# terasum/mythril

Measured on AMD Instinct MI355X. Metric: constraint-evals/sec, higher is better.
Workload: dtype u32; 1 GPU; synthetic config 5: 10000 random 256-bit constraint tapes x 67108864 assignments per GPU, throughput mode; variant=plain, tapes=10000, rows_per_gpu=67108864, rows_total=67108864, vars=4, mode=count_all, engine=jit, short_circuit=True, parallelism=dp1 (row shards, all-reduce of per-tape results)

## Files before the change

### mythril_amd/csrc/jit.cpp

```cpp
#include "jit.h"

#include <math.h>
#include <stdarg.h>
#include <stdio.h>
#include <string.h>

#include <algorithm>
#include <atomic>
#include <climits>
#include <cstdlib>
#include <functional>
#include <stdexcept>
#include <string>
#include <thread>
#include <unordered_map>
#include <vector>

namespace mh {
namespace jit {

namespace {

struct Fail {
    std::string why;
// ... 64 lines not shown
uint32_t prefix_mask(uint32_t m) { int t = top_bit(m); return t < 0 ? 0u : ((2u << t) - 1u); }

class Emitter {
public:
    Emitter(const SsaTape& st, const std::vector<uint32_t>& pool, uint32_t n_vars,
            const Options& opt, const std::vector<uint8_t>* check = nullptr,
            std::vector<double>* insn_cost = nullptr)
        : st_(st), pool_(pool), n_vars_(n_vars), opt_(opt), check_(check),
          insn_cost_(insn_cost) {}

    TapeCode run();

private:
    SsaTape st_;
    const std::vector<uint32_t>& pool_;
    uint32_t n_vars_;
    Options opt_;
    const std::vector<uint8_t>* check_;
    std::vector<double>* insn_cost_;
    bool sc_used_ = false;
    std::vector<MI> code_;
    std::vector<Val> vals_;
    std::vector<int> last_;
    std::vector<uint8_t> dem_;
    int vref_[512] = {};
    uint32_t vbase_ = 0, vmax_ = 0, vhigh_ = 0;
    int pref_[N_BOOL_PAIRS] = {};
    uint32_t kstage_ = 0;
    uint32_t n_valu_ = 0, n_wide_ = 0, n_salu_ = 0;
    uint32_t n_valu_cold_ = 0;
    int cold_ = 0;
    bool calls_div_ = false;
    bool calls_divw_ = false;
    bool uses_lds_ = false;
    bool calls_kec_ = false;
    int cur_op_ = -1;
    int live_vreg_ = -1;
public:
    static uint64_t op_valu[256], op_wide[256], op_count[256];
    int div_ = 0;
    bool divw_ = false;
private:

    void emit(uint16_t op, std::initializer_list<Opnd> ops, bool e64 = false) {
        MI m;
        m.op = op;
        m.e64 = e64 ? 1 : 0;
        m.tag = cur_op_ >= 0 ? (uint8_t)cur_op_ : 0xFF;
        int i = 0;
        for (const Opnd& o : ops) m.o[i++] = o;
        code_.push_back(m);
        if (op <= M_V_CMP_LE_F64) {
            ++n_valu_;
            if (cold_ > 0) ++n_valu_cold_;
            const bool wide = e64 || op == M_V_ADD_CO || op == M_V_ADDC_CO || op == M_V_SUB_CO ||
                              op == M_V_SUBB_CO || op == M_V_SUBREV_CO || op == M_V_SUBBREV_CO ||
                              op == M_V_OR3 || op == M_V_ALIGNBIT || op == M_V_MAD_U64_U32 ||
                              op == M_V_LSHL_ADD || op == M_V_PERM || op == M_V_BFI ||
                              op == M_V_LSHLREV || op == M_V_LSHRREV || op == M_V_ASHRREV ||
                              (op >= M_V_CMP_EQ && op <= M_V_CMP_GT_I32) || op >= M_V_CVT_F64_U32 ||
                              op == M_V_RCP_F32 || op == M_V_CMP_GT_F32 || op == M_V_CMP_LE_F32;
            if (wide) ++n_wide_;
            if (cur_op_ >= 0) { ++op_valu[cur_op_]; op_wide[cur_op_] += wide; }
        } else if (op <= M_S_CMP_LT_U32) {
            ++n_salu_;
        }
    }

    uint32_t next_lbl_ = 0x1000;

    uint32_t valloc() {
        for (uint32_t r = vbase_; r < vmax_; ++r)
            if (vref_[r] == 0) {
                vref_[r] = 1;
// ... 1186 lines not shown
    const uint32_t rbase = kind == 1 ? R_DR : R_DQ;
    int path = 0;
    if (div_ >= 1 && ny >= 1 && nx < ny && kind < 4) {
        if (kind < 2 && B.l[ny - 1].is_c()) {
            Val R;
            R.defined = true;
            for (int k = 0; k < 8; ++k) {
                if (!((dm >> k) & 1)) continue;
                R.l[k] = kind == 1 && k < nx ? A.l[k] : Limb::C(0);
                if (R.l[k].is_r()) vretain(R.l[k].v);
            }
            vals_[d] = R;
            return;
        }
        path = B.l[ny - 1].is_r() ? 1 : 0;
        if (kind & 1)
            for (int k = 0; k < nx; ++k)
                if (A.l[k].is_r() && A.l[k].v >= rbase && A.l[k].v < rbase + 8 &&
                    A.l[k].v != rbase + (uint32_t)k)
                    path = 0;
    } else if (div_ >= 3 && nx == 8 && ny == 8 && (kind == 0 || kind == 2)) {
        path = 3;
    }
    uint32_t l_join = 0;
    if (path) {
        const uint32_t l_cold = next_lbl_++;
        l_join = next_lbl_++;
        if (path == 1) div_short_dividend(A, B, kind, nx, dm, cur, l_cold);
        else div_small_quotient(A, B, kind, dm, cur, l_cold);
        emit(M_S_BRANCH, {LBL(l_join)});
        emit(M_LABEL, {LBL(l_cold)});
        ++cold_;
    }
    if (kind < 2) {
        for (int k = 0; k < 8; ++k) emit(M_V_MOV, {V(R_DY + k), src(B.l[k])});
        for (int k = 0; k < 8; ++k) emit(M_V_MOV, {V(R_DR + k), src(A.l[k])});
    } else {
        auto sign_of = [&](const Val& X, uint32_t sreg) {
            if (X.l[7].is_c()) emit(M_V_MOV, {V(sreg), IMM((X.l[7].v >> 31) ? ~0u : 0u)});
            else emit(M_V_ASHRREV, {V(sreg), IMM(31), V(X.l[7].v)});
        };
        auto load_abs = [&](uint32_t base, uint32_t sreg, const Val& X) {
            bool allc = true;
            for (int k = 0; k < 8; ++k) allc = allc && X.l[k].is_c();
            const bool known = X.l[7].is_c(), neg = known && (X.l[7].v >> 31);
            if (allc) {
                uint32_t c[8];
                uint64_t borrow = neg ? 1 : 0;
                for (int k = 0; k < 8; ++k) {
                    const uint64_t t = (uint64_t)(neg ? ~X.l[k].v : X.l[k].v) + borrow;
                    c[k] = (uint32_t)t;
                    borrow = t >> 32;
                }
                for (int k = 0; k < 8; ++k) emit(M_V_MOV, {V(base + k), IMM(c[k])});
                return;
            }
            if (known && !neg) {
                for (int k = 0; k < 8; ++k) emit(M_V_MOV, {V(base + k), src(X.l[k])});
                return;
            }
            for (int k = 0; k < 8; ++k) {
                if (X.l[k].is_c(0)) emit(M_V_MOV, {V(base + k), V(sreg)});
                else emit(M_V_XOR, {V(base + k), src(X.l[k]), V(sreg)});
            }
            emit(M_V_SUB_CO, {V(base), VCC(), V(base), V(sreg)});
            for (int k = 1; k < 8; ++k)
                emit(M_V_SUBB_CO, {V(base + k), VCC(), V(base + k), V(sreg), VCC()});
// ... 4 lines not shown
        load_abs(R_DR, R_SX, A);
    }
    int wny = 0;
    bool wconst = false;
    uint32_t yc[8] = {0};
    if (divw_ && path == 0) {
        wconst = true;
        for (int k = 0; k < 8; ++k) wconst = wconst && B.l[k].is_c();
        if (wconst) {
            const bool neg = kind >= 2 && (B.l[7].v >> 31);
            uint64_t carry = neg ? 1 : 0;
            for (int k = 0; k < 8; ++k) {
                const uint64_t t = (uint64_t)(neg ? ~B.l[k].v : B.l[k].v) + carry;
                yc[k] = (uint32_t)t;
                carry = t >> 32;
            }
            wny = 8;
            while (wny > 0 && !yc[wny - 1]) --wny;
        } else {
            wny = ny;
        }
        if (wny < 1 || wny > 7 || nx < wny) wny = 0;
    }
    if (wny) {
        const int j0 = nx - wny;
        calls_divw_ = true;
        emit(M_S_MOV_B32, {S(S_DIV_KIND), IMM(kind | (uint32_t)((wconst ? 64 : 0) + 8 * wny + j0) << 3)});
        emit(M_S_MOV_B32, {S(S_DIV_DUMMY), IMM(kind)});
        if (wconst) {
            const uint64_t rb = div_recip_bits(yc, wny);
            emit(M_S_MOV_B32, {S(S_DIV_F64K), IMM((uint32_t)rb)});
            emit(M_S_MOV_B32, {S(S_DIV_F64K + 1), IMM((uint32_t)(rb >> 32))});
        }
    } else {
        emit(M_S_MOV_B32, {S(S_DIV_KIND), IMM(kind)});
    }
    emit(M_CALL_DIV, {IMM((uint32_t)code_.size())});
    if (path) {
        --cold_;
        emit(M_LABEL, {LBL(l_join)});
    }
    int nr = path == 1 && (kind & 1) ? nx : 8;
    if (wny && wconst && kind < 2) nr = kind == 1 ? wny : nx - wny + 1;
    Val& R = out(d);
    for (int k = 0; k < 8; ++k)
        if ((dm >> k) & 1) R.l[k] = k < nr ? Limb::R(rbase + k) : Limb::C(0);
}

void Emitter::div_undecided(Opnd decided, int cur) {
    const Opnd t = S(S_DIV_TM, 2);
    emit(M_S_ANDN2_B64, {t, S(S_VALID, 2), decided});
    const int lv = live_vreg_;
    if (check_ && lv >= 0 && vals_[lv].defined && vals_[lv].is_bool && vals_[lv].bconst < 0 &&
        last_[lv] > cur)
        emit(M_S_AND_B64, {t, t, P(vals_[lv].pair)});
}

void Emitter::div_short_dividend(const Val& A, const Val& B, uint32_t kind, int nx, uint32_t dm,
                                 int cur, uint32_t l_cold) {
    int ny = 8;
    while (!B.l[ny - 1].is_r()) --ny;
    const uint32_t top = B.l[ny - 1].v;
    if (kind < 2) {
        emit(M_V_CMP_NE, {VCC(), IMM(0), V(top)});
    } else {
        emit(M_V_ASHRREV, {V(R_T1), IMM(31), V(top)});
        emit(M_V_XOR, {V(R_T1), V(top), V(R_T1)});
        emit(M_V_CMP_NE, {VCC(), IMM(0), V(R_T1)});
    }
// ... 881 lines not shown
                emit(M_S_BRANCH, {LBL(LBL_SC_END)});
                emit(M_LABEL, {LBL(LBL_SC_SKIP)});
                emit(M_S_MOV_B64, {S(S_RES, 2), IMM(0)});
                emit(M_LABEL, {LBL(LBL_SC_END)});
            }
            for (int k = 0; k < 8; ++k) { tc.root_limbs[k] = ~0u; tc.root_const[k] = 0; }
        } else {
            uint32_t acc = ~0u, cacc = 0;
            for (int k = 0; k < 8; ++k) {
                const Limb l = root.l[k];
                if (l.is_c()) { cacc |= l.v; tc.root_limbs[k] = ~0u; tc.root_const[k] = l.v; continue; }
                tc.root_limbs[k] = l.v;
                tc.root_const[k] = 0;
                if (acc == ~0u) { acc = valloc(); emit(M_V_MOV, {V(acc), V(l.v)}); }
                else emit(M_V_OR, {V(acc), V(l.v), V(acc)});
            }
            if (cacc) emit(M_S_MOV_B64, {S(S_RES, 2), IMM(~0u)});
            else if (acc == ~0u) emit(M_S_MOV_B64, {S(S_RES, 2), IMM(0)});
            else {
                emit(M_V_CMP_NE, {VCC(), IMM(0), V(acc)});
                emit(M_S_MOV_B64, {S(S_RES, 2), VCC()});
            }
        }
        tc.ok = true;
    } catch (const Fail& f) {
        tc.ok = false;
        tc.why = f.why;
        code_.clear();
    }
    tc.code.swap(code_);
    tc.max_vgpr = vhigh_;
    tc.calls_div = calls_div_;
    tc.calls_divw = calls_divw_;
    tc.uses_lds = uses_lds_;
    tc.calls_kec = calls_kec_;
    tc.n_valu = n_valu_;
    tc.n_valu_wide = n_wide_;
    tc.n_salu = n_salu_;
    return tc;
}

struct OpInfo {
    const char* name;
};
const char* op_name(uint16_t op) {
    switch (op) {
        case M_V_MOV: return "v_mov_b32";
        case M_V_ADD_U32: return "v_add_u32";
        case M_V_SUB_U32: return "v_sub_u32";
        case M_V_SUBREV_U32: return "v_subrev_u32";
        case M_V_ADD_CO: return "v_add_co_u32";
        case M_V_ADDC_CO: return "v_addc_co_u32";
        case M_V_SUB_CO: return "v_sub_co_u32";
        case M_V_SUBB_CO: return "v_subb_co_u32";
        case M_V_SUBREV_CO: return "v_subrev_co_u32";
        case M_V_SUBBREV_CO: return "v_subbrev_co_u32";
        case M_V_AND: return "v_and_b32";
        case M_V_OR: return "v_or_b32";
        case M_V_XOR: return "v_xor_b32";
        case M_V_NOT: return "v_not_b32";
        case M_V_XNOR: return "v_xnor_b32";
        case M_V_OR3: return "v_or3_b32";
        case M_V_ALIGNBIT: return "v_alignbit_b32";
        case M_V_LSHLREV: return "v_lshlrev_b32";
        case M_V_LSHRREV: return "v_lshrrev_b32";
        case M_V_ASHRREV: return "v_ashrrev_i32";
// ... 90 lines not shown
        for (const Opnd& x : ops) m.o[i++] = x;
        o.push_back(m);
    };
    auto L = [&](uint32_t id) { E(M_LABEL, {LBL(id)}); };
    auto Yr = [](int k) { return V(R_DY + k); };
    auto Rr = [](int k) { return V(R_DR + k); };
    auto Xr = [](int k) { return V(R_DQ + k); };
    const Opnd FY = V(R_FY, 2), FR = V(R_FR, 2), FC = V(R_FC, 2), FT = V(R_FT, 2);
    const Opnd CARRY = V(R_CARRY, 2), MAD = V(R_MAD, 2);
    const Opnd C = V(R_C), T1 = V(R_T1), SX = V(R_SX), SY = V(R_SY);
    const Opnd YNZ = S(S_DIV_YNZ, 2), DUMMY = S(S_DIV_DUMMY, 2), MSK = S(S_DIV_MSK, 2),
               TM = S(S_DIV_TM, 2), K64 = S(S_DIV_F64K, 2), KIND = S(S_DIV_KIND);
    const Opnd K64LO = S(S_DIV_F64K), K64HI = S(S_DIV_F64K + 1);
    enum : uint32_t { L_UNS = 1, L_DONE, L_TOP3, L_CONV, L_ZQ, L_NOZQ, L_STEP0 = 10, L_NONEG0 = 20, L_NOGE0 = 30, L_WB = 40,
                      L_SDIV, L_SREM, L_SMOD, L_NARROW = 50, L_NNEG0 = 60, L_NGE0 = 70,
                      L_NOYZ = 80, L_CZ0 = 90, L_RLT = 100, L_RLTD, L_YSLOW, L_YDONE, L_TOPALL,
                      L_F32 = 110, L_F32OK, L_STEP0_BODY };
    auto to_f64 = [&](Opnd dst, Opnd (*limb)(int)) {
        E(M_S_MOV_B32, {K64LO, IMM(0)});
        E(M_S_MOV_B32, {K64HI, IMM(0x41f00000u)});
        E(M_V_CVT_F64_U32, {dst, limb(7)});
        for (int k = 6; k >= 0; --k) {
            E(M_V_CVT_F64_U32, {FT, limb(k)});
            E(M_V_FMA_F64, {dst, dst, K64, FT});
        }
    };
    auto Rl = [](int k) { return V(R_DR + k); };
    auto Yl = [](int k) { return V(R_DY + k); };
    const Opnd KEEP = S(S_DIV_DUMMY);
    enum : uint32_t { L_WHEAD = 128, L_WSEC, L_WCONST, L_WVAR = 136 , L_WCON = 144 ,
                      L_WOK = 152 , L_WZQ = 160 ,
                      L_WSTEP = 256 , L_WNONEG = 384, L_WNOGE = 512,
                      L_WTREE = 640 };
    L(L_WHEAD);
    E(M_S_CMP_LT_U32, {KIND, IMM(64)});
    E(M_S_CBRANCH_SCC1, {LBL(L_UNS)});
    {
        uint32_t tree = L_WTREE;
        std::function<void(int, int, uint32_t, uint32_t)> pick = [&](int lo, int hi, uint32_t c,
                                                                      uint32_t base) {
            if (lo == hi) {
                E(M_S_BRANCH, {LBL(base + (uint32_t)lo)});
                return;
            }
            const int mid = (lo + hi + 1) / 2;
            const uint32_t l = tree++;
            E(M_S_CMP_LT_U32, {KIND, IMM((64 * c + 8 * (uint32_t)mid) << 3)});
            E(M_S_CBRANCH_SCC0, {LBL(l)});
            pick(lo, mid - 1, c, base);
            L(l);
            pick(mid, hi, c, base);
        };
        E(M_S_CMP_LT_U32, {KIND, IMM(64u << 3)});
        E(M_S_CBRANCH_SCC0, {LBL(L_WCONST)});
        pick(1, 7, 0, L_WVAR);
        L(L_WCONST);
        pick(1, 7, 1, L_WCON);
    }
    L(L_UNS);
    E(M_S_CMP_EQ_U32, {KIND, IMM(0)});
    E(M_S_CBRANCH_SCC1, {LBL(L_ZQ)});
    E(M_S_CMP_EQ_U32, {KIND, IMM(2)});
    E(M_S_CBRANCH_SCC0, {LBL(L_NOZQ)});
    L(L_ZQ);
    for (int k = 0; k < 8; ++k) E(M_V_MOV, {Xr(k), IMM(0)});
    L(L_NOZQ);
// ... 17 lines not shown
    E(M_V_CMP_LT, {VCC(), Rr(7), Yr(7)});
    E(M_S_BRANCH, {LBL(L_RLTD)});
    L(L_RLT);
    E(M_V_SUB_CO, {T1, VCC(), Rr(0), Yr(0)});
    for (int k = 1; k < 8; ++k) E(M_V_SUBB_CO, {T1, VCC(), Rr(k), Yr(k), VCC()});
    L(L_RLTD);
    E(M_S_ANDN2_B64, {MSK, YNZ, VCC()});
    E(M_S_CMP_EQ_U64, {MSK, IMM(0)});
    E(M_S_CBRANCH_SCC1, {LBL(L_DONE)});
    E(M_S_CMP_EQ_U64, {TM, IMM(0)});
    E(M_S_CBRANCH_SCC1, {LBL(L_NARROW)});
    auto recip = [&]() {
        E(M_V_RCP_F64, {FC, FY});
        E(M_S_NOP, {IMM(1)});
        E(M_V_FMA_F64, {FT, NEG(FY), FC, FONE()});
        E(M_V_FMA_F64, {FC, FC, FT, FC});
        E(M_V_FMA_F64, {FT, NEG(FY), FC, FONE()});
        E(M_V_FMA_F64, {FY, FC, FT, FC});
    };
    auto top3_f64 = [&](Opnd dst, Opnd (*limb)(int)) {
        E(M_S_MOV_B32, {K64LO, IMM(0)});
        E(M_S_MOV_B32, {K64HI, IMM(0x41f00000u)});
        E(M_V_CVT_F64_U32, {dst, limb(7)});
        for (int k = 6; k >= 5; --k) {
            E(M_V_CVT_F64_U32, {FT, limb(k)});
            E(M_V_FMA_F64, {dst, dst, K64, FT});
        }
        E(M_S_MOV_B32, {K64HI, IMM((uint32_t)(1023 + 160) << 20)});
        E(M_V_MUL_F64, {dst, dst, K64});
    };
    E(M_V_CMP_NE, {VCC(), IMM(0), Yr(7)});
    E(M_S_ANDN2_B64, {TM, MSK, VCC()});
    E(M_S_CBRANCH_SCC0, {LBL(L_F32)});
    to_f64(FY, Yl);
    recip();
    to_f64(FR, Rl);
    E(M_S_BRANCH, {LBL(L_CONV)});
    L(L_F32);
    E(M_S_MOV_B32, {K64LO, IMM(0x4f800000u)});
    E(M_V_CVT_F32_U32, {V(R_FT), Rr(7)});
    E(M_V_CVT_F32_U32, {V(R_FT + 1), Rr(6)});
    E(M_V_FMA_F32, {V(R_FR), V(R_FT), K64LO, V(R_FT + 1)});
    E(M_V_CVT_F32_U32, {V(R_FT), Yr(7)});
    E(M_V_CVT_F32_U32, {V(R_FT + 1), Yr(6)});
    E(M_V_FMA_F32, {V(R_FY), V(R_FT), K64LO, V(R_FT + 1)});
    E(M_V_RCP_F32, {V(R_FY), V(R_FY)});
    E(M_S_NOP, {IMM(1)});
    E(M_V_MUL_F32, {V(R_FC), V(R_FR), V(R_FY)});
    E(M_V_CMP_GT_F32, {VCC(), IMM(0x44800000u), V(R_FC)});
    E(M_S_ANDN2_B64, {TM, MSK, VCC()});
    E(M_S_CBRANCH_SCC0, {LBL(L_F32OK)});
    E(M_V_CMP_NE, {VCC(), IMM(0), Yr(7)});
    E(M_S_BRANCH, {LBL(L_TOP3)});
    L(L_F32OK);
    E(M_V_CVT_U32_F32, {C, V(R_FC)});
    E(M_V_CNDMASK, {C, IMM(0), C, MSK}, true);
    E(M_V_FRACT_F32, {V(R_FT), V(R_FC)});
    E(M_V_CMP_LE_F32, {VCC(), IMM(0x3f7f8000u), V(R_FT)});
    E(M_S_AND_B64, {TM, VCC(), MSK});
    E(M_S_BRANCH, {LBL(L_STEP0_BODY)});
    L(L_TOP3);
    top3_f64(FY, Yl);
    recip();
    E(M_S_CMP_EQ_U64, {VCC(), IMM(0xFFFFFFFFu)});
    E(M_S_CBRANCH_SCC1, {LBL(L_TOPALL)});
    E(M_V_CNDMASK, {V(R_FY), IMM(0), V(R_FY), MSK}, true);
// ... 321 lines not shown
            E(M_S_MOV_B64, {MSK, VCC()});
            E(M_S_CMP_EQ_U64, {MSK, IMM(0)});
            E(M_S_CBRANCH_SCC1, {LBL(L_WNONEG + id)});
            for (int k = 0; k < ny; ++k) {
                E(M_V_CNDMASK, {T1, IMM(0), Yr(k), MSK}, true);
                if (k == 0) E(M_V_ADD_CO, {Rr(j), VCC(), Rr(j), T1});
                else E(M_V_ADDC_CO, {Rr(j + k), VCC(), Rr(j + k), T1, VCC()});
            }
            if (top <= 7) E(M_V_ADDC_CO, {Rr(top), VCC(), IMM(0), Rr(top), VCC()});
            E(M_V_CNDMASK, {T1, IMM(0), IMM(1), MSK}, true);
            E(M_V_SUB_U32, {C, C, T1});
            L(L_WNONEG + id);
            E(M_S_CMP_EQ_U64, {TM, IMM(0)});
            E(M_S_CBRANCH_SCC1, {LBL(L_WNOGE + id)});
            E(M_V_SUB_CO, {T1, VCC(), Rr(j), Yr(0)});
            for (int k = 1; k < ny; ++k) E(M_V_SUBB_CO, {T1, VCC(), Rr(j + k), Yr(k), VCC()});
            if (top <= 7) E(M_V_SUBBREV_CO, {T1, VCC(), IMM(0), Rr(top), VCC()});
            E(M_S_ANDN2_B64, {MSK, YNZ, VCC()});
            E(M_S_CMP_EQ_U64, {MSK, IMM(0)});
            E(M_S_CBRANCH_SCC1, {LBL(L_WNOGE + id)});
            for (int k = 0; k < ny; ++k) {
                E(M_V_CNDMASK, {T1, IMM(0), Yr(k), MSK}, true);
                if (k == 0) E(M_V_SUB_CO, {Rr(j), VCC(), Rr(j), T1});
                else E(M_V_SUBB_CO, {Rr(j + k), VCC(), Rr(j + k), T1, VCC()});
            }
            if (top <= 7) E(M_V_SUBBREV_CO, {Rr(top), VCC(), IMM(0), Rr(top), VCC()});
            E(M_V_CNDMASK, {T1, IMM(0), IMM(1), MSK}, true);
            E(M_V_ADD_U32, {C, C, T1});
            L(L_WNOGE + id);
            E(M_V_MOV, {Xr(j), C});
        }
        leave(L_DONE);
    }
    return o;
}

namespace {
const uint64_t kKeccakRC[24] = {
    0x0000000000000001ull, 0x0000000000008082ull, 0x800000000000808Aull, 0x8000000080008000ull,
    0x000000000000808Bull, 0x0000000080000001ull, 0x8000000080008081ull, 0x8000000000008009ull,
    0x000000000000008Aull, 0x0000000000000088ull, 0x0000000080008009ull, 0x000000008000000Aull,
    0x000000008000808Bull, 0x800000000000008Bull, 0x8000000000008089ull, 0x8000000000008003ull,
    0x8000000000008002ull, 0x8000000000000080ull, 0x000000000000800Aull, 0x800000008000000Aull,
    0x8000000080008081ull, 0x8000000000008080ull, 0x0000000080000001ull, 0x8000000080008008ull};
const int kRhoPi[24][2] = {{10, 1}, {7, 3},   {11, 6},  {17, 10}, {18, 15}, {3, 21},
                           {5, 28}, {16, 36}, {8, 45},  {21, 55}, {24, 2},  {4, 14},
                           {15, 27}, {23, 41}, {19, 56}, {13, 8},  {12, 25}, {2, 43},
                           {20, 62}, {14, 18}, {22, 39}, {9, 61},  {6, 20},  {1, 44}};
}

namespace {

void kec_theta_states(uint8_t* comp) {
    uint8_t c[5] = {0}, d[5];
    for (int i = 0; i < 25; ++i) c[i % 5] ^= comp[i];
    for (int x = 0; x < 5; ++x) d[x] = c[(x + 4) % 5] ^ c[(x + 1) % 5];
    for (int i = 0; i < 25; ++i) comp[i] ^= d[i % 5];
}

void kec_rhopi_states(uint8_t* comp) {
    uint8_t cur = comp[1];
    for (int step = 0; step < 24; ++step) {
        const int dst = kRhoPi[step][0];
        const uint8_t t = comp[dst];
        comp[dst] = cur;
        cur = t;
// ... 324 lines not shown
    char b[512];
    va_list ap;
    va_start(ap, fmt);
    vsnprintf(b, sizeof b, fmt, ap);
    va_end(ap);
    out += b;
    out += '\n';
}

}

Module build_module(const std::vector<const TapeCode*>& codes,
                    const std::vector<uint32_t>& tape_ids, uint32_t n_vars, bool values,
                    uint32_t group_bytes) {
    Module m;
    std::string& o = m.text;
    uint32_t cur = 0, first = 0;
    for (uint32_t i = 0; i < codes.size(); ++i) {
        const uint32_t b = code_bytes(*codes[i]) + 96;
        if (i > first && (cur + b > group_bytes || i - first >= 64)) {
            m.group_first.push_back(first);
            m.group_count.push_back(i - first);
            first = i;
            cur = 0;
        }
        cur += b;
    }
    if (first < codes.size()) {
        m.group_first.push_back(first);
        m.group_count.push_back((uint32_t)codes.size() - first);
    }
    const uint32_t n_pin = pinned_cols(n_vars);
    uint32_t maxv = R_COL0 + 8 * n_pin;
    bool any_div = false, any_divw = false, any_lds = false, any_kec = false;
    for (const TapeCode* tc : codes) {
        maxv = std::max(maxv, tc->max_vgpr);
        any_div |= tc->calls_div;
        any_divw |= tc->calls_divw;
        any_lds |= tc->uses_lds;
        any_kec |= tc->calls_kec;
    }
    if (any_kec) maxv = std::max<uint32_t>(maxv, R_TEMP_KEC);
    if (any_div) maxv = std::max<uint32_t>(maxv, R_TEMP0);
    maxv = std::max<uint32_t>(maxv, 8);
    static const uint32_t pad = [] {
        const char* e = std::getenv("MH_JIT_PAD_VGPR");
        const uint32_t v = e ? (uint32_t)atoi(e) : 0u;
        return v <= 512 ? v : 0u;
    }();
    maxv = std::max(maxv, pad);
    maxv = (maxv + 7) & ~7u;
    m.max_vgpr = maxv;
    m.n_sgpr = S_NEXT_FREE;

    line(o, ".amdgcn_target \"amdgcn-amd-amdhsa--gfx950\"");
    line(o, ".amdhsa_code_object_version 5");
    line(o, ".text");
    line(o, ".globl mh_jit");
    line(o, ".p2align 8");
    line(o, ".type mh_jit,@function");
    line(o, "mh_jit:");
    line(o, "s_load_dwordx16 s[4:19], s[0:1], 0x0");
    line(o, "s_load_dwordx4 s[20:23], s[0:1], 0x40");
    line(o, "v_and_b32 v1, 63, v0");
    line(o, "v_lshrrev_b32 v2, 6, v0");
    line(o, "s_nop 1");
    line(o, "v_readfirstlane_b32 s24, v2");
    if (any_lds) {
        line(o, "v_mul_u32_u24 v%u, 0x%x, v2", R_LDS, LDS_WAVE_BYTES);
        line(o, "v_lshl_add_u32 v%u, v1, 2, v%u", R_LDS, R_LDS);
        line(o, "v_mov_b32 v5, 0");
// ... 121 lines not shown
                line(o, "s_cbranch_scc1 mh_g%zue%u_nc", g, t);
                line(o, "s_mov_b64 exec, 1");
                line(o, "s_nop 1");
                line(o, "v_mov_b32 v6, s34");
                line(o, "v_mov_b32 v7, 0");
                line(o, "v_mov_b32 v5, 0x%x", id * 8u);
                line(o, "global_atomic_add_x2 v5, v[6:7], s[16:17]");
                line(o, "s_mov_b64 exec, -1");
                line(o, "mh_g%zue%u_nc:", g, t);
                line(o, "v_readlane_b32 s34, v4, %u", t);
                line(o, "s_cmp_eq_u32 s34, 0");
                line(o, "s_cbranch_scc1 mh_g%zue%u_nf", g, t);
                line(o, "s_sub_u32 s34, s34, 1");
                line(o, "s_add_u32 s34, s34, s12");
                line(o, "s_addc_u32 s35, s13, 0");
                line(o, "s_mov_b64 exec, 1");
                line(o, "s_nop 1");
                line(o, "v_mov_b32 v6, s34");
                line(o, "v_mov_b32 v7, s35");
                line(o, "v_mov_b32 v5, 0x%x", id * 8u);
                line(o, "global_atomic_umin_x2 v5, v[6:7], s[14:15]");
                line(o, "s_mov_b64 exec, -1");
                line(o, "mh_g%zue%u_nf:", g, t);
            }
        }
        line(o, "s_endpgm");
    }
    if (any_div) {
        line(o, ".p2align 6");
        line(o, "mh_div:");
        std::vector<MI> dv;
        bool keep = true;
        for (const MI& mi : div_routine()) {
            if (mi.op == M_LABEL && !any_divw) {
                if (mi.o[0].v == 128 || mi.o[0].v == 129) keep = false;
                else if (mi.o[0].v == 1) keep = true;
            }
            if (keep) dv.push_back(mi);
        }
        print_list(dv, "mh_dv", o);
    }
    if (any_kec) {
        line(o, ".p2align 6");
        line(o, "mh_kec:");
        print_list(kec_routine().code, "mh_kc", o);
    }
    line(o, ".Lmh_jit_end:");
    line(o, ".size mh_jit, .Lmh_jit_end-mh_jit");
    line(o, ".rodata");
    line(o, ".p2align 6");
    line(o, ".amdhsa_kernel mh_jit");
    line(o, "  .amdhsa_group_segment_fixed_size %u", any_lds ? (uint32_t)LDS_WG_BYTES : 0u);
    line(o, "  .amdhsa_private_segment_fixed_size 0");
    line(o, "  .amdhsa_kernarg_size %u", (uint32_t)sizeof(KernArgs));
    line(o, "  .amdhsa_user_sgpr_count 2");
    line(o, "  .amdhsa_user_sgpr_kernarg_segment_ptr 1");
    line(o, "  .amdhsa_system_sgpr_workgroup_id_x 1");
    line(o, "  .amdhsa_system_sgpr_workgroup_id_y 1");
    line(o, "  .amdhsa_system_vgpr_workitem_id 0");
    line(o, "  .amdhsa_next_free_vgpr %u", maxv);
    line(o, "  .amdhsa_next_free_sgpr %u", (uint32_t)S_NEXT_FREE);
    line(o, "  .amdhsa_accum_offset %u", (maxv + 3) & ~3u);
    line(o, "  .amdhsa_reserve_vcc 1");
    line(o, "  .amdhsa_ieee_mode 1");
    line(o, "  .amdhsa_dx10_clamp 1");
    line(o, ".end_amdhsa_kernel");
    line(o, ".amdgpu_metadata");
    line(o, "---");
    line(o, "amdhsa.kernels:");
// ... 280 lines not shown
                if (!(w.second && k == 0) && m.o[k].n > 1 && touches(m.o[k], x)) pair_read = true;
            }
            if (w.second && x >= w.first && x < w.first + w.second) {
                ok = w.second == 1 && w.first == x && !tt;
                break;
            }
            if (tt || pair_read) break;
        }
        if (!ok) continue;
        code[q].o[0].v = t;
        for (size_t i = q + 1; i < p; ++i)
            for (int k = 0; k < 5; ++k)
                if (code[i].o[k].k == O_V && code[i].o[k].n == 1 && code[i].o[k].v == x)
                    code[i].o[k].v = t;
        gone[p] = 1;
        ++removed;
    }
    if (removed) {
        std::vector<MI> out;
        out.reserve(code.size() - removed);
        for (size_t i = 0; i < code.size(); ++i)
            if (!gone[i]) out.push_back(code[i]);
        code.swap(out);
    }
    return removed;
}

}

static std::atomic<uint64_t> g_sc_fallbacks{0};

static int stage_level() {
    const char* e = std::getenv("MH_JIT_STAGE");
    return e ? std::min(5, std::max(0, atoi(e))) : 5;
}

static int div_level() {
    const char* s = std::getenv("MH_JIT_STAGE");
    if (s && atoi(s) <= 0) return 0;
    const char* e = std::getenv("MH_JIT_DIV");
    return e ? std::min(3, std::max(0, atoi(e))) : 3;
}

uint64_t sc_fallbacks(bool reset) {
    return reset ? g_sc_fallbacks.exchange(0) : g_sc_fallbacks.load();
}

TapeCode emit_tape(const SsaTape& st, const std::vector<uint32_t>& pool, uint32_t n_vars,
                   const Options& opt) {
    TapeCode tc = emit_tape_body(st, pool, n_vars, opt);
    if (tc.ok && opt.coalesce) {
        const uint32_t r = coalesce_div_moves(tc.code);
        tc.n_valu -= r;
    }
    return tc;
}

TapeCode emit_tape_body(const SsaTape& st, const std::vector<uint32_t>& pool, uint32_t n_vars,
                        const Options& opt) {
    const int dlevel = div_level();
    const bool divw = dlevel > 0 && stage_level() >= 5;
    std::vector<double> cost;
    Emitter e(st, pool, n_vars, opt, nullptr, opt.short_circuit ? &cost : nullptr);
    e.div_ = opt.short_circuit ? 0 : dlevel;
    e.divw_ = !opt.short_circuit && divw;
    TapeCode tc0 = e.run();
    if (opt.short_circuit) {
        SsaTape sc;
        std::vector<uint8_t> check;
        if (schedule_conjuncts(st, pool, opt.sample_rows, tc0.ok ? &cost : nullptr, sc, check)) {
            const int level = opt.stage >= 0 ? opt.stage : stage_level();
            if (level > 0) {
                Emitter e2(sc, pool, n_vars, opt, &check);
                e2.stage_ = level;
                e2.div_ = dlevel;
                e2.divw_ = divw;
                TapeCode tc = e2.run();
                if (tc.ok && !e2.stage_rejected_.empty()) {
                    std::vector<uint8_t> skip((size_t)sc.n_vregs, 0);
                    for (int d : e2.stage_rejected_) skip[(size_t)d] = 1;
                    Emitter e3(sc, pool, n_vars, opt, &check);
                    e3.stage_ = level;
                    e3.div_ = dlevel;
                    e3.divw_ = divw;
                    e3.stage_skip_ = &skip;
                    tc = e3.run();
                }
                if (tc.ok && level >= 4 && tc.max_vgpr > Options().max_vgpr) {
                    Options o3 = opt;
                    o3.stage = 3;
                    TapeCode t3 = emit_tape_body(st, pool, n_vars, o3);
                    if (t3.ok && (t3.max_vgpr + 7) / 8 < (tc.max_vgpr + 7) / 8) return t3;
                }
                if (tc.ok) return tc;
            }
            Emitter e2(sc, pool, n_vars, opt, &check);
            e2.div_ = dlevel;
            e2.divw_ = divw;
            TapeCode tc = e2.run();
            if (tc.ok) return tc;
            g_sc_fallbacks.fetch_add(1, std::memory_order_relaxed);
        }
        if (dlevel > 0 && tc0.ok && tc0.calls_div) {
            Emitter e4(st, pool, n_vars, opt);
            e4.div_ = dlevel;
            e4.divw_ = divw;
            TapeCode tc = e4.run();
            if (tc.ok) return tc;
        }
    }
    return tc0;
}

}
}
```

### mythril_amd/csrc/jit.h

```cpp
#pragma once
#include <stdint.h>

#include <string>
#include <vector>

#include "compile.h"

namespace mh {
namespace jit {

enum OKind : uint8_t { O_NONE, O_V, O_S, O_VCC, O_IMM, O_LABEL, O_EXEC, O_FONE  };

struct Opnd {
    uint8_t k = O_NONE;
    uint8_t n = 1;
    uint8_t neg = 0;
    uint32_t v = 0;
};

inline Opnd V(uint32_t r, uint8_t n = 1) { Opnd o; o.k = O_V; o.v = r; o.n = n; return o; }
inline Opnd S(uint32_t r, uint8_t n = 1) { Opnd o; o.k = O_S; o.v = r; o.n = n; return o; }
inline Opnd VCC() { Opnd o; o.k = O_VCC; o.n = 2; return o; }
inline Opnd EXEC() { Opnd o; o.k = O_EXEC; o.n = 2; return o; }
inline Opnd IMM(uint32_t x) { Opnd o; o.k = O_IMM; o.v = x; return o; }
// ... 33 lines not shown
    M_DS_READ_B32,
    M_S_WAITCNT_LGKM,
    M_LOADCOL,
    M_S_WAITCNT_VM,
    M_NUM_OPS
};

struct MI {
    uint16_t op;
    uint8_t e64 = 0;
    uint8_t tag = 0xFF;
    Opnd o[5];
};

constexpr uint32_t kMaxPinnedCols = 4;
inline uint32_t pinned_cols(uint32_t n_vars) { return n_vars <= kMaxPinnedCols ? n_vars : 0u; }

enum : uint32_t {
    R_LDS = 7,
    R_COL0 = 8,
    R_DIV0 = 40,
    R_DY = 40, R_DR = 48, R_DQ = 56, R_FY = 64, R_FR = 66, R_FC = 68, R_FT = 70,
    R_CARRY = 72, R_MAD = 74, R_C = 76, R_T1 = 77, R_SX = 78, R_SY = 79,
    R_TEMP0 = 80,
    R_TEMP_NODIV = 40,
    R_KEC0 = 40,
    N_KEC_REGS = 62,
    R_TEMP_KEC = 102,
    S_VALID = 30,
    S_RES = 32,
    S_SCRATCH = 34,
    S_BOOL0 = 40, N_BOOL_PAIRS = 16,
    S_KSTAGE = 72, N_KSTAGE = 4,
    S_DIV_RA = 76, S_DIV_TGT = 78, S_DIV_KIND = 80, S_DIV_YNZ = 82, S_DIV_DUMMY = 84,
    S_DIV_MSK = 86, S_DIV_TM = 88, S_DIV_F64K = 90,
    S_PERM_SEL = 92,
    S_NEXT_FREE = 93,
};

enum : uint32_t {
    LDS_D = 8, LDS_WORDS = 25, LDS_WAVE_BYTES = LDS_WORDS * 256, LDS_WG_BYTES = 4 * LDS_WAVE_BYTES,
};

struct TapeCode {
    bool ok = false;
    std::string why;
    std::vector<MI> code;
    uint32_t max_vgpr = 0;
    bool calls_div = false;
    bool calls_divw = false;
    bool uses_lds = false;
    bool calls_kec = false;
    bool root_bool = true;
    uint32_t root_limbs[8];
    uint32_t root_const[8];
    uint32_t n_valu = 0, n_valu_wide = 0, n_salu = 0;
    uint64_t alg_ops = 0;
};

struct Options {
    uint32_t max_vgpr = 128;
    uint32_t max_vgpr_keccak = 168;
    bool short_circuit = true;
    uint32_t sample_rows = 256;
    bool coalesce = true;
    int stage = -1;
    bool assemble = true;
};

bool schedule_conjuncts(const SsaTape& st, const std::vector<uint32_t>& pool,
                        uint32_t sample_rows, const std::vector<double>* insn_cost, SsaTape& out,
                        std::vector<uint8_t>& check);

TapeCode emit_tape(const SsaTape& st, const std::vector<uint32_t>& pool, uint32_t n_vars,
                   const Options& opt);
TapeCode emit_tape_body(const SsaTape& st, const std::vector<uint32_t>& pool, uint32_t n_vars,
                        const Options& opt);

std::vector<MI> div_routine();

struct KecCode {
    std::vector<MI> code;
    uint32_t out[8];
// ... 67 lines not shown
```

Before: 469.6 billion evals/s.

## Add fast-entry signed division path and per-divisor-width dispatch in JIT div routine

Adds a new division entry layer (stage 6, on by default) to the JIT-generated 256-bit division routine. For signed division of full-width register operands, a raw path estimates a small quotient with f32 reciprocal arithmetic on the top limbs and applies it with a multiply-subtract. Rows whose estimate is unsafe fall back to negating operands and taking the unsigned path. A second layer probes the divisor's top nonzero limb at runtime and jumps into the existing per-width f64 reciprocal step code, aiming to avoid the generic full-width conversion and long division. This adds code size, branches and SGPR use (a flag register carved from the old KIND pair), with some risk of correctness or divergence cost.

```diff
diff --git a/mythril_amd/csrc/jit.cpp b/mythril_amd/csrc/jit.cpp
--- a/mythril_amd/csrc/jit.cpp
+++ b/mythril_amd/csrc/jit.cpp
@@ -120,6 +120,7 @@
     int cold_ = 0;
     bool calls_div_ = false;
     bool calls_divw_ = false;
+    bool calls_dive_ = false;
     bool uses_lds_ = false;
     bool calls_kec_ = false;
     int cur_op_ = -1;
@@ -128,6 +129,7 @@
     static uint64_t op_valu[256], op_wide[256], op_count[256];
     int div_ = 0;
     bool divw_ = false;
+    int dive_ = 0;
 private:
 
     void emit(uint16_t op, std::initializer_list<Opnd> ops, bool e64 = false) {
@@ -1380,7 +1382,18 @@
         emit(M_LABEL, {LBL(l_cold)});
         ++cold_;
     }
-    if (kind < 2) {
+    const bool raw = (dive_ & 1) && path == 0 && kind == 3 && nx == 8 && ny == 8 && A.l[7].is_r() &&
+                     B.l[7].is_r();
+    if (raw) {
+        emit(M_S_MOV_B64, {S(S_DIV_TM, 2), S(S_VALID, 2)});
+        const int lv = live_vreg_;
+        if (check_ && lv >= 0 && vals_[lv].defined && vals_[lv].is_bool && vals_[lv].bconst < 0 &&
+            last_[lv] > cur)
+            emit(M_S_AND_B64, {S(S_DIV_TM, 2), S(S_DIV_TM, 2), P(vals_[lv].pair)});
+        emit(M_V_ASHRREV, {V(R_SY), IMM(31), V(B.l[7].v)});
+        emit(M_V_ASHRREV, {V(R_SX), IMM(31), V(A.l[7].v)});
+    }
+    if (kind < 2 || raw) {
         for (int k = 0; k < 8; ++k) emit(M_V_MOV, {V(R_DY + k), src(B.l[k])});
         for (int k = 0; k < 8; ++k) emit(M_V_MOV, {V(R_DR + k), src(A.l[k])});
     } else {
@@ -1451,9 +1464,13 @@
             emit(M_S_MOV_B32, {S(S_DIV_F64K), IMM((uint32_t)rb)});
             emit(M_S_MOV_B32, {S(S_DIV_F64K + 1), IMM((uint32_t)(rb >> 32))});
         }
+    } else if (raw) {
+        emit(M_S_MOV_B32, {S(S_DIV_KIND), IMM(kind | (128u + (uint32_t)std::max(top_bit(dm), 0)) << 3)});
+        emit(M_S_MOV_B32, {S(S_DIV_FLAG6), IMM((dive_ & 2) ? 1u : 0u)});
     } else {
-        emit(M_S_MOV_B32, {S(S_DIV_KIND), IMM(kind)});
-    }
+        emit(M_S_MOV_B32, {S(S_DIV_KIND), IMM((dive_ & 2) ? kind | 2048u : kind)});
+    }
+    if (dive_) calls_dive_ = true;
     emit(M_CALL_DIV, {IMM((uint32_t)code_.size())});
     if (path) {
         --cold_;
@@ -2401,6 +2418,7 @@
     tc.max_vgpr = vhigh_;
     tc.calls_div = calls_div_;
     tc.calls_divw = calls_divw_;
+    tc.calls_dive = calls_dive_;
     tc.uses_lds = uses_lds_;
     tc.calls_kec = calls_kec_;
     tc.n_valu = n_valu_;
@@ -2557,6 +2575,19 @@
                       L_WOK = 152 , L_WZQ = 160 ,
                       L_WSTEP = 256 , L_WNONEG = 384, L_WNOGE = 512,
                       L_WTREE = 640 };
+    enum : uint32_t { L_SRAW = 113, L_SCOLD, L_BNO, L_BGO , L_EOLD = 123, L_SFULL,
+                      L_EHEAD = 200, L_ESEC, L_BSEC, L_BEND };
+    const Opnd FLAG6 = S(S_DIV_FLAG6);
+    L(L_EHEAD);
+    E(M_S_CMP_LT_U32, {KIND, IMM(1024)});
+    E(M_S_CBRANCH_SCC1, {LBL(L_EOLD)});
+    E(M_S_CMP_LT_U32, {KIND, IMM(2048)});
+    E(M_S_CBRANCH_SCC1, {LBL(L_SRAW)});
+    E(M_S_AND_B64, {S(S_DIV_KIND, 2), S(S_DIV_KIND, 2), IMM(7)});
+    E(M_S_MOV_B32, {FLAG6, IMM(1)});
+    E(M_S_BRANCH, {LBL(L_UNS)});
+    L(L_EOLD);
+    E(M_S_MOV_B32, {FLAG6, IMM(0)});
     L(L_WHEAD);
     E(M_S_CMP_LT_U32, {KIND, IMM(64)});
     E(M_S_CBRANCH_SCC1, {LBL(L_UNS)});
@@ -2640,6 +2671,41 @@
     E(M_V_CMP_NE, {VCC(), IMM(0), Yr(7)});
     E(M_S_ANDN2_B64, {TM, MSK, VCC()});
     E(M_S_CBRANCH_SCC0, {LBL(L_F32)});
+    L(L_BSEC);
+    E(M_S_CMP_EQ_U32, {FLAG6, IMM(1)});
+    E(M_S_CBRANCH_SCC0, {LBL(L_BNO)});
+    E(M_S_CMP_LG_U64, {VCC(), IMM(0)});
+    E(M_S_CBRANCH_SCC1, {LBL(L_BNO)});
+    for (int k = 6; k >= 1; --k) {
+        E(M_V_CMP_NE, {VCC(), IMM(0), Yr(k)});
+        E(M_S_CMP_EQ_U64, {VCC(), IMM(0xFFFFFFFFu)});
+        E(M_S_CBRANCH_SCC1, {LBL(L_BGO + (uint32_t)k)});
+        E(M_S_CMP_LG_U64, {VCC(), IMM(0)});
+        E(M_S_CBRANCH_SCC1, {LBL(L_BNO)});
+    }
+    E(M_S_BRANCH, {LBL(L_BNO)});
+    for (int k = 6; k >= 1; --k) {
+        const int ny = k + 1, jmax = 8 - ny, wl = std::min(ny, 3);
+        L(L_BGO + (uint32_t)k);
+        E(M_S_MOV_B32, {S(S_DIV_DUMMY), KIND});
+        E(M_S_MOV_B32, {K64LO, IMM(0)});
+        E(M_S_MOV_B32, {K64HI, IMM(0x41f00000u)});
+        E(M_V_CVT_F64_U32, {FY, Yr(ny - 1)});
+        for (int i = ny - 2; i >= ny - wl; --i) {
+            E(M_V_CVT_F64_U32, {FT, Yr(i)});
+            E(M_V_FMA_F64, {FY, FY, K64, FT});
+        }
+        recip();
+        E(M_S_MOV_B64, {YNZ, IMM(0xFFFFFFFFu)});
+        for (int j = jmax; j >= 1; --j) {
+            E(M_V_CMP_NE, {VCC(), IMM(0), Rr(j + ny - 1)});
+            E(M_S_CMP_LG_U64, {VCC(), IMM(0)});
+            E(M_S_CBRANCH_SCC1, {LBL(L_WSTEP + 16 * (uint32_t)ny + (uint32_t)j)});
+        }
+        E(M_S_BRANCH, {LBL(L_WSTEP + 16 * (uint32_t)ny)});
+    }
+    L(L_BNO);
+    L(L_BEND);
     to_f64(FY, Yl);
     recip();
     to_f64(FR, Rl);
@@ -3027,6 +3093,74 @@
         }
         leave(L_DONE);
     }
+    L(L_ESEC);
+    L(L_SRAW);
+    {
+        const Opnd K32 = K64LO, KT = K64HI, ONE = S(S_DIV_YNZ);
+        E(M_V_XOR, {V(R_MAD), Yr(7), SY});
+        E(M_V_CMP_NE, {VCC(), IMM(0), V(R_MAD)});
+        E(M_S_ANDN2_B64, {DUMMY, TM, VCC()});
+        E(M_S_CBRANCH_SCC1, {LBL(L_SCOLD)});
+        E(M_V_XOR, {V(R_MAD + 1), Yr(6), SY});
+        E(M_V_XOR, {V(R_CARRY), Rr(7), SX});
+        E(M_V_XOR, {V(R_CARRY + 1), Rr(6), SX});
+        E(M_S_MOV_B32, {K32, IMM(0x4f800000u)});
+        E(M_V_CVT_F32_U32, {V(R_FT), V(R_CARRY)});
+        E(M_V_CVT_F32_U32, {V(R_FT + 1), V(R_CARRY + 1)});
+        E(M_V_FMA_F32, {V(R_FR), V(R_FT), K32, V(R_FT + 1)});
+        E(M_V_CVT_F32_U32, {V(R_FT), V(R_MAD)});
+        E(M_V_CVT_F32_U32, {V(R_FT + 1), V(R_MAD + 1)});
+        E(M_V_FMA_F32, {V(R_FY), V(R_FT), K32, V(R_FT + 1)});
+        E(M_V_RCP_F32, {V(R_FY), V(R_FY)});
+        E(M_S_NOP, {IMM(1)});
+        E(M_V_MUL_F32, {V(R_FC), V(R_FR), V(R_FY)});
+        E(M_V_CMP_GT_F32, {VCC(), IMM(0x44800000u), V(R_FC)});
+        E(M_S_MOV_B64, {MSK, VCC()});
+        E(M_V_FRACT_F32, {V(R_FT), V(R_FC)});
+        E(M_S_MOV_B32, {KT, IMM(0x35800000u)});
+        E(M_V_FMA_F32, {T1, V(R_FC), KT, KT});
+        E(M_V_CMP_GT_F32, {VCC(), T1, V(R_FT)});
+        E(M_S_MOV_B64, {DUMMY, VCC()});
+        E(M_V_CMP_LE_F32, {VCC(), IMM(0x3f800000u), V(R_FC)});
+        E(M_S_AND_B64, {DUMMY, DUMMY, VCC()});
+        E(M_S_ANDN2_B64, {MSK, MSK, DUMMY});
+        E(M_S_MOV_B32, {ONE, IMM(0x3f800000u)});
+        E(M_V_FMA_F32, {T1, T1, ONE, V(R_FT)});
+        E(M_V_CMP_LE_F32, {VCC(), IMM(0x3f800000u), T1});
+        E(M_S_ANDN2_B64, {MSK, MSK, VCC()});
+        E(M_S_ANDN2_B64, {DUMMY, TM, MSK});
+        E(M_S_CBRANCH_SCC1, {LBL(L_SCOLD)});
+        E(M_V_CVT_U32_F32, {C, V(R_FC)});
+        E(M_V_XOR, {T1, SX, SY});
+        E(M_V_CMP_NE, {VCC(), IMM(0), T1});
+        auto limb = [&](int k, bool last) {
+            E(M_V_MAD_U64_U32, {MAD, DUMMY, C, Yr(k), k ? CARRY : IMM(0)});
+            if (k == 0 && !last) E(M_V_MOV, {V(R_CARRY + 1), IMM(0)});
+            if (!last) E(M_V_MOV, {V(R_CARRY), V(R_MAD + 1)});
+            E(M_V_XOR, {V(R_MAD), V(R_MAD), T1});
+            E(M_V_SUBB_CO, {Xr(k), VCC(), Rr(k), V(R_MAD), VCC()});
+        };
+        E(M_S_CMP_LT_U32, {KIND, IMM((128u + 7u) << 3)});
+        E(M_S_CBRANCH_SCC0, {LBL(L_SFULL)});
+        for (int k = 0; k < 7; ++k) {
+            limb(k, false);
+            E(M_S_CMP_LT_U32, {KIND, IMM((128u + (uint32_t)k + 1u) << 3)});
+            E(M_S_CBRANCH_SCC1, {LBL(L_WB)});
+        }
+        E(M_S_BRANCH, {LBL(L_WB)});
+        L(L_SFULL);
+        for (int k = 0; k < 8; ++k) limb(k, k == 7);
+        E(M_S_BRANCH, {LBL(L_WB)});
+        L(L_SCOLD);
+        for (int k = 0; k < 8; ++k) E(M_V_XOR, {Yr(k), Yr(k), SY});
+        E(M_V_SUB_CO, {Yr(0), VCC(), Yr(0), SY});
+        for (int k = 1; k < 8; ++k) E(M_V_SUBB_CO, {Yr(k), VCC(), Yr(k), SY, VCC()});
+        for (int k = 0; k < 8; ++k) E(M_V_XOR, {Rr(k), Rr(k), SX});
+        E(M_V_SUB_CO, {Rr(0), VCC(), Rr(0), SX});
+        for (int k = 1; k < 8; ++k) E(M_V_SUBB_CO, {Rr(k), VCC(), Rr(k), SX, VCC()});
+        E(M_S_MOV_B32, {KIND, IMM(3)});
+        E(M_S_BRANCH, {LBL(L_UNS)});
+    }
     return o;
 }
 
@@ -3417,11 +3551,12 @@
     }
     const uint32_t n_pin = pinned_cols(n_vars);
     uint32_t maxv = R_COL0 + 8 * n_pin;
-    bool any_div = false, any_divw = false, any_lds = false, any_kec = false;
+    bool any_div = false, any_divw = false, any_dive = false, any_lds = false, any_kec = false;
     for (const TapeCode* tc : codes) {
         maxv = std::max(maxv, tc->max_vgpr);
         any_div |= tc->calls_div;
-        any_divw |= tc->calls_divw;
+        any_divw |= tc->calls_divw || tc->calls_dive;
+        any_dive |= tc->calls_dive;
         any_lds |= tc->uses_lds;
         any_kec |= tc->calls_kec;
     }
@@ -3609,9 +3744,14 @@
         std::vector<MI> dv;
         bool keep = true;
         for (const MI& mi : div_routine()) {
-            if (mi.op == M_LABEL && !any_divw) {
-                if (mi.o[0].v == 128 || mi.o[0].v == 129) keep = false;
-                else if (mi.o[0].v == 1) keep = true;
+            if (mi.op == M_LABEL) {
+                const uint32_t l = mi.o[0].v;
+                if (l == 128 || l == 129) keep = any_divw;
+                else if (l == 1) keep = true;
+                else if (l >= 200 && l <= 203) {
+                    keep = l == 203 ? true : any_dive;
+                    continue;
+                }
             }
             if (keep) dv.push_back(mi);
         }
@@ -3958,7 +4098,7 @@
 
 static int stage_level() {
     const char* e = std::getenv("MH_JIT_STAGE");
-    return e ? std::min(5, std::max(0, atoi(e))) : 5;
+    return e ? std::min(6, std::max(0, atoi(e))) : 6;
 }
 
 static int div_level() {
@@ -3966,6 +4106,11 @@
     if (s && atoi(s) <= 0) return 0;
     const char* e = std::getenv("MH_JIT_DIV");
     return e ? std::min(3, std::max(0, atoi(e))) : 3;
+}
+
+static int entry_layers() {
+    const char* e = std::getenv("MH_JIT_ENTRY");
+    return e ? (atoi(e) & 3) : 3;
 }
 
 uint64_t sc_fallbacks(bool reset) {
@@ -3986,10 +4131,12 @@
                         const Options& opt) {
     const int dlevel = div_level();
     const bool divw = dlevel > 0 && stage_level() >= 5;
+    const int dive = dlevel > 0 && stage_level() >= 6 ? entry_layers() : 0;
     std::vector<double> cost;
     Emitter e(st, pool, n_vars, opt, nullptr, opt.short_circuit ? &cost : nullptr);
     e.div_ = opt.short_circuit ? 0 : dlevel;
     e.divw_ = !opt.short_circuit && divw;
+    e.dive_ = opt.short_circuit ? 0 : dive;
     TapeCode tc0 = e.run();
     if (opt.short_circuit) {
         SsaTape sc;
@@ -4001,6 +4148,7 @@
                 e2.stage_ = level;
                 e2.div_ = dlevel;
                 e2.divw_ = divw;
+                e2.dive_ = dive;
                 TapeCode tc = e2.run();
                 if (tc.ok && !e2.stage_rejected_.empty()) {
                     std::vector<uint8_t> skip((size_t)sc.n_vregs, 0);
@@ -4009,6 +4157,7 @@
                     e3.stage_ = level;
                     e3.div_ = dlevel;
                     e3.divw_ = divw;
+                    e3.dive_ = dive;
                     e3.stage_skip_ = &skip;
                     tc = e3.run();
                 }
@@ -4023,6 +4172,7 @@
             Emitter e2(sc, pool, n_vars, opt, &check);
             e2.div_ = dlevel;
             e2.divw_ = divw;
+            e2.dive_ = dive;
             TapeCode tc = e2.run();
             if (tc.ok) return tc;
             g_sc_fallbacks.fetch_add(1, std::memory_order_relaxed);
@@ -4031,6 +4181,7 @@
             Emitter e4(st, pool, n_vars, opt);
             e4.div_ = dlevel;
             e4.divw_ = divw;
+            e4.dive_ = dive;
             TapeCode tc = e4.run();
             if (tc.ok) return tc;
         }
diff --git a/mythril_amd/csrc/jit.h b/mythril_amd/csrc/jit.h
--- a/mythril_amd/csrc/jit.h
+++ b/mythril_amd/csrc/jit.h
@@ -89,7 +89,9 @@
     S_SCRATCH = 34,
     S_BOOL0 = 40, N_BOOL_PAIRS = 16,
     S_KSTAGE = 72, N_KSTAGE = 4,
-    S_DIV_RA = 76, S_DIV_TGT = 78, S_DIV_KIND = 80, S_DIV_YNZ = 82, S_DIV_DUMMY = 84,
+    S_DIV_RA = 76, S_DIV_TGT = 78, S_DIV_KIND = 80,
+    S_DIV_FLAG6 = 81,
+    S_DIV_YNZ = 82, S_DIV_DUMMY = 84,
     S_DIV_MSK = 86, S_DIV_TM = 88, S_DIV_F64K = 90,
     S_PERM_SEL = 92,
     S_NEXT_FREE = 93,
@@ -106,6 +108,7 @@
     uint32_t max_vgpr = 0;
     bool calls_div = false;
     bool calls_divw = false;
+    bool calls_dive = false;
     bool uses_lds = false;
     bool calls_kec = false;
     bool root_bool = true;
```

New measurement: 474.9 billion evals/s, median of 6. 1.01x the previous value.
